# wfus/Fully-Homomorphic-Image-Processing

Hardware: AMD Instinct MI355X
Metric: encrypted 8x8 blocks/sec (homomorphic DCT+quant) (higher is better)
Workload: dtype f64

## Files before the change

### fully-homomorphic-image-processing_amd/csrc/dct_fused.hip

```cpp
#include "internal.h"

#include <cstdlib>

#include "fp64_core.h"

#pragma clang fp contract(off)

namespace {
using namespace fp64;

template <int L, int LE> struct Shape {
    static constexpr int N = 1 << L, E = 1 << LE, TP = N >> LE, NP = (L + LE - 1) / LE, LDS_WORDS = N + (N >> LE);
};
__host__ __device__ constexpr int g_lo(int L, int LE, int p) { return (L - LE * p - LE) < 0 ? 0 : (L - LE * p - LE); }
__host__ __device__ constexpr int g_stages(int L, int LE, int p) { return (L - LE * p) > LE ? LE : (L - LE * p); }
template <int LO, int LE> __device__ __forceinline__ int g_index(int tid, int r) {
    return ((tid >> LO) << (LO + LE)) | (r << LO) | (tid & ((1 << LO) - 1));
}
template <int LO, int LE> __device__ __forceinline__ int g_pad(int j) { return j + ((j >> (LO + LE)) << LO); }

template <int L, int LE, int P> struct PassTw {
    static constexpr int LO = g_lo(L, LE, P), S = g_stages(L, LE, P), NTW = (1 << LE) - 1;
    static constexpr int rb(int u) { return (L - 1 - (LE * P + u)) - LO; }
    static constexpr int count(int u) { return 1 << (LE - 1 - rb(u)); }
// ... 131 lines not shown
}
template <int L, int LE, int M, bool BIG, int P = Shape<L, LE>::NP - 1>
__device__ __forceinline__ void ntt_inv(double (&x)[M][1 << LE], double (&w)[(1 << LE) - 1], const double *__restrict__ itw, double p, double pinv,
                                        double *lds, int tid, int &phase) {
    if constexpr (P > 0) {
        double wn[(1 << LE) - 1];
        if (LE >= 4) load_tw<L, LE, P - 1>(wn, itw, tid);
        inv_pass<L, LE, P, M>(x, w, 0.0, p, pinv);
        if (LE < 4) load_tw<L, LE, P - 1>(wn, itw, tid);
        if constexpr (BIG) {
#pragma unroll
            for (int m = 0; m < M; m++)
#pragma unroll
                for (int r = 0; r < (1 << LE); r++) x[m][r] = red(x[m][r], p, pinv);
        }
        transpose<L, LE, g_lo(L, LE, P), g_lo(L, LE, P - 1), M>(x, lds, tid, phase);
        ntt_inv<L, LE, M, BIG, P - 1>(x, wn, itw, p, pinv, lds, tid, phase);
    } else {
        inv_pass<L, LE, P, M>(x, w, itw[0], p, pinv);
    }
}

constexpr double PACK_BIAS = 6755399441055744.0;
template <int E, int TP>
__device__ __forceinline__ void store_packed(char *__restrict__ ob, u32 vo, u32 so, const double (&x)[E]) {
    static_assert(E == 8, "packed layout is defined for 8 values per thread");
    u32 lo[8], hi[8];
#pragma unroll
    for (int r = 0; r < 8; r++) {
        const double t = x[r] + PACK_BIAS;
        lo[r] = (u32)__double2loint(t);
        hi[r] = (u32)__double2hiint(t);
    }
#pragma unroll
    for (int q = 0; q < 4; q++) *(u64 *)(ob + (size_t)(so + q * TP * 8) + vo) = (u64)lo[2 * q] | ((u64)lo[2 * q + 1] << 32);
    u32 h[2];
#pragma unroll
    for (int g = 0; g < 2; g++) {
        const u32 p01 = __builtin_amdgcn_perm(hi[4 * g + 1], hi[4 * g + 0], 0x0c0c0400u);
        const u32 p23 = __builtin_amdgcn_perm(hi[4 * g + 3], hi[4 * g + 2], 0x0c0c0400u);
        h[g] = __builtin_amdgcn_perm(p23, p01, 0x05040100u);
    }
    *(u64 *)(ob + (size_t)(so + 4 * TP * 8) + vo) = (u64)h[0] | ((u64)h[1] << 32);
}
typedef __attribute__((address_space(3))) void lc_lptr;
template <int NT>
__device__ __forceinline__ void stage_consts(gwin_t w, u32 voff, u32 soff, u32 cstride_bytes, double *stg) {
#pragma unroll
    for (int i0 = 0; i0 < NT; i0 += 2) {
        const int i = (i0 + 1 < NT) ? i0 : NT - 2;
        __builtin_amdgcn_raw_ptr_buffer_load_lds(w, (lc_lptr *)(stg + i * 64), 16, voff, soff + (u32)i * cstride_bytes, 0, 0);
    }
}

template <int L, int LE, bool BIG, int HALF, bool PACK, bool LDSC>
__device__ __forceinline__ void rows_body(const u64 *__restrict__ in, double *__restrict__ mid, const double *__restrict__ consts,
                                          const double *__restrict__ tw, const Work &wk, double p, double pinv, u32 k, double *lds) {
    using SH = Shape<L, LE>;
    constexpr int N = SH::N, TP = SH::TP, E = SH::E, NC = HalfC<HALF>::NC, FIRST = HalfC<HALF>::FIRST;
    const int tid = threadIdx.x;
    const size_t poly_words = (size_t)k * N, ct_words = 2 * poly_words;
    const size_t base = ((size_t)wk.blk * 64 + 8 * wk.line) * ct_words + (size_t)wk.poly * poly_words + (size_t)wk.prime * N;
    const gwin_t win_in = gwin(in + base), win_mid = gwin(mid + base);
    const u32 vo = (u32)tid * 8u, ctb = (u32)(ct_words * 8);
    double w0[E - 1];
    load_tw<L, LE, 0>(w0, tw, tid);
    double x[4][E];
    u64 ra[2][E], rb[2][E];
    auto issue = [&](int m) {
#pragma unroll
        for (int r = 0; r < E; r++) {
            ra[m & 1][r] = gld_u64(win_in, vo, (u32)m * ctb + r * TP * 8);
            rb[m & 1][r] = gld_u64(win_in, vo, (u32)(7 - m) * ctb + r * TP * 8);
        }
    };
// ... 45 lines not shown
    }
#pragma unroll
    for (int r = 0; r < E; r++) {
        double c[9];
        if constexpr (LDSC) {
            if (r + 1 < E) stage_consts<NC>(win_c, svoff, (r + 1) * TP * 8, csb, stg + ((r + 1) & 1) * NC * 64);
            if (r + 1 < E) asm volatile("s_waitcnt vmcnt(%0)" ::"n"(NDMA) : "memory");
            else asm volatile("s_waitcnt vmcnt(0)" ::: "memory");
            const double *sr = stg + (r & 1) * NC * 64 + lane;
#pragma unroll
            for (int i = 0; i < NC; i++) c[i] = sr[i * 64];
        } else {
        if (LE < 4) fetch(r);
#pragma unroll
        for (int i = 0; i < NC; i++) c[i] = cn[i];
        if (LE >= 4 && r + 1 < E) fetch(r + 1);
        }
        line_half<HALF>(x[0][r], x[1][r], x[2][r], x[3][r], c, p, pinv);
        if (BIG) {
#pragma unroll
            for (int m = 0; m < 4; m++) x[m][r] = red(x[m][r], p, pinv);
        } else if (PACK && HALF == 0) {
            x[0][r] = red(x[0][r], p, pinv);
            x[2][r] = red(x[2][r], p, pinv);
        }
        if constexpr (LDSC) asm volatile("" ::"v"(x[0][r]), "v"(x[1][r]), "v"(x[2][r]), "v"(x[3][r]) : "memory");
    }
#pragma unroll
    for (int m = 0; m < 4; m++) {
        const u32 so = (u32)(2 * m + HALF) * ctb;
        if constexpr (PACK) {
            store_packed<E, TP>((char *)(mid + base), vo, so, x[m]);
        } else {
#pragma unroll
            for (int r = 0; r < E; r++) gst_f64(win_mid, vo, so + r * TP * 8, x[m][r]);
        }
    }
}

__host__ __device__ constexpr int occ_waves(int tp, int lds_words) {
    return ((2 * lds_words * 16 <= 160 * 1024) ? 2 : 1) * tp / 256 < 1 ? 1 : ((2 * lds_words * 16 <= 160 * 1024) ? 2 : 1) * tp / 256;
}
template <int L, int LE> struct Occ { static constexpr int W = occ_waves(Shape<L, LE>::TP, Shape<L, LE>::LDS_WORDS); };

template <int L, int LE, bool BIG, bool PACK, bool LDSC>
__global__ __launch_bounds__((Shape<L, LE>::TP), (Occ<L, LE>::W)) void k_dct_rows(const u64 *__restrict__ in, double *__restrict__ mid,
                                                                  const double *__restrict__ consts, const double *__restrict__ tw_all,
                                                                  const Modulus *__restrict__ mods, u32 k) {
    __shared__ double lds[2 * Shape<L, LE>::LDS_WORDS];
    const Work wk = decode(blockIdx.x, k);
    const double p = (double)mods[wk.prime].q, pinv = 1.0 / p;
    const double *tw = tw_all + (size_t)wk.prime * Shape<L, LE>::N;
    if (wk.half) rows_body<L, LE, BIG, 1, PACK, LDSC>(in, mid, consts, tw, wk, p, pinv, k, lds);
    else rows_body<L, LE, BIG, 0, PACK, LDSC>(in, mid, consts, tw, wk, p, pinv, k, lds);
}

template <int L, int LE, bool BIG, int HALF, bool PACK>
__device__ __forceinline__ void cols_body(const double *__restrict__ mid, u64 *__restrict__ out, const double *__restrict__ consts,
                                          const double *__restrict__ itw, const Work &wk, double p, double pinv, u32 k, double *lds) {
    using SH = Shape<L, LE>;
    constexpr int N = SH::N, TP = SH::TP, E = SH::E, NC = HalfC<HALF>::NC, FIRST = HalfC<HALF>::FIRST;
    constexpr int LASTP = SH::NP - 1;
    const int tid = threadIdx.x;
    const size_t poly_words = (size_t)k * N, ct_words = 2 * poly_words;
    const size_t base = ((size_t)wk.blk * 64 + wk.line) * ct_words + (size_t)wk.poly * poly_words + (size_t)wk.prime * N;
    const size_t cstride = (size_t)k * N;
    const gwin_t win_mid = gwin(mid + base), win_out = gwin(out + base);
    const gwin_t win_c = gwin(consts + (size_t)FIRST * cstride + (size_t)wk.prime * N);
    const gwin_t win_s = gwin(consts + (size_t)(12 + 8 * HALF + wk.line) * cstride + (size_t)wk.prime * N);
    const u32 vo = (u32)tid * 8u, rsb = (u32)(ct_words * 64), csb = (u32)(cstride * 8);
    const double pbias = p + 4503599627370496.0;
    double cn[9], sn[4];
    auto fetch = [&](int r) {
#pragma unroll
        for (int i = 0; i < NC; i++) cn[i] = gld_f64(win_c, vo, (u32)i * csb + r * TP * 8);
#pragma unroll
        for (int m = 0; m < 4; m++) sn[m] = gld_f64(win_s, vo, (u32)(16 * m) * csb + r * TP * 8);
    };
    double wl[E - 1];
    if constexpr (!PACK) {
        fetch(0);
        load_tw<L, LE, LASTP>(wl, itw, tid);
    }
    double x[4][E];
    if constexpr (PACK) {
        u64 wa[4][5], wb[4][5];
#pragma unroll
        for (int m = 0; m < 4; m++) {
#pragma unroll
            for (int q = 0; q < 5; q++) {
                wa[m][q] = gld_u64(win_mid, vo, (u32)m * rsb + q * TP * 8);
                wb[m][q] = gld_u64(win_mid, vo, (u32)(7 - m) * rsb + q * TP * 8);
            }
        }
#pragma unroll
        for (int m = 0; m < 4; m++) {
#pragma unroll
            for (int r = 0; r < E; r++) {
                const u32 la = (r & 1) ? (u32)(wa[m][r >> 1] >> 32) : (u32)wa[m][r >> 1];
                const u32 lb = (r & 1) ? (u32)(wb[m][r >> 1] >> 32) : (u32)wb[m][r >> 1];
                const u32 hwa = (r & 4) ? (u32)(wa[m][4] >> 32) : (u32)wa[m][4], hwb = (r & 4) ? (u32)(wb[m][4] >> 32) : (u32)wb[m][4];
                const double ta = __hiloint2double((int)(0x43380000u + (u32)(int)(signed char)(hwa >> (8 * (r & 3)))), (int)la);
                const double tb = __hiloint2double((int)(0x43380000u + (u32)(int)(signed char)(hwb >> (8 * (r & 3)))), (int)lb);
                x[m][r] = HALF ? ta - tb : ta + (tb - 2.0 * PACK_BIAS);
            }
        }
    } else {
#pragma unroll
        for (int m = 0; m < 4; m++) {
#pragma unroll
            for (int r = 0; r < E; r++) {
                const double A = gld_f64(win_mid, vo, (u32)m * rsb + r * TP * 8), B = gld_f64(win_mid, vo, (u32)(7 - m) * rsb + r * TP * 8);
                x[m][r] = HALF ? A - B : A + B;
            }
        }
    }
    if constexpr (PACK) load_tw<L, LE, LASTP>(wl, itw, tid);
#pragma unroll
    for (int r = 0; r < E; r++) {
        double c[9], sc[4];
        if (PACK) fetch(r);
#pragma unroll
        for (int i = 0; i < NC; i++) c[i] = cn[i];
#pragma unroll
        for (int m = 0; m < 4; m++) sc[m] = sn[m];
        if (!PACK && r + 1 < E) fetch(r + 1);
        line_half<HALF>(x[0][r], x[1][r], x[2][r], x[3][r], c, p, pinv);
        double y[4] = {x[0][r], x[1][r], x[2][r], x[3][r]};
        mmv<4>(y, sc, p, pinv);
#pragma unroll
        for (int m = 0; m < 4; m++) x[m][r] = y[m];
    }
    int phase = 0;
    ntt_inv<L, LE, 4, BIG>(x, wl, itw, p, pinv, lds, tid, phase);
#pragma unroll
    for (int m = 0; m < 4; m++) {
#pragma unroll
        for (int r = 0; r < E; r++) gst_u64(win_out, vo, (u32)(2 * m + HALF) * rsb + r * TP * 8, f64_to_residue(x[m][r], pbias));
    }
}

template <int L, int LE, bool BIG, bool PACK>
__global__ __launch_bounds__((Shape<L, LE>::TP), (Occ<L, LE>::W)) void k_dct_cols(const double *__restrict__ mid, u64 *__restrict__ out,
                                                                  const double *__restrict__ consts, const double *__restrict__ itw_all,
                                                                  const Modulus *__restrict__ mods, u32 k) {
    __shared__ double lds[2 * Shape<L, LE>::LDS_WORDS];
    const Work wk = decode(blockIdx.x, k);
    const double p = (double)mods[wk.prime].q, pinv = 1.0 / p;
    const double *itw = itw_all + (size_t)wk.prime * Shape<L, LE>::N;
    if (wk.half) cols_body<L, LE, BIG, 1, PACK>(mid, out, consts, itw, wk, p, pinv, k, lds);
    else cols_body<L, LE, BIG, 0, PACK>(mid, out, consts, itw, wk, p, pinv, k, lds);
}

template <int L, int LE>
__global__ __launch_bounds__((Shape<L, LE>::TP), (Occ<L, LE>::W)) void k_dct_one_launch(const u64 *__restrict__ in, double *__restrict__ mid, u64 *__restrict__ out,
                                                                        const double *__restrict__ consts, const double *__restrict__ tw_all,
                                                                        const double *__restrict__ itw_all, const Modulus *__restrict__ mods, u32 k,
                                                                        u32 n_blocks, u32 dist, u32 *__restrict__ arrived, u32 *__restrict__ err) {
    __shared__ double lds[2 * Shape<L, LE>::LDS_WORDS];
    const u32 xcd = blockIdx.x & 7, seq = blockIdx.x >> 3, chunk = seq >> 5, r = seq & 31;
    const bool is_row = r < 16;
    const long j = is_row ? (long)chunk : (long)chunk - (long)(dist & 0xffffu);
    const u32 n_units = n_blocks * 2 * k;
    if (j < 0) return;
    const u64 g = (u64)j * 8 + xcd;
    if (g >= n_units) return;
    Work wk;
    wk.prime = (u32)(g / (n_blocks * 2));
    const u32 rem = (u32)(g - (u64)wk.prime * n_blocks * 2);
    wk.blk = rem >> 1;
    wk.poly = rem & 1;
    wk.line = (r & 15) >> 1;
    wk.half = r & 1;
    const double p = (double)mods[wk.prime].q, pinv = 1.0 / p;
    if (is_row) {
        const double *tw = tw_all + (size_t)wk.prime * Shape<L, LE>::N;
        if (wk.half) rows_body<L, LE, false, 1, true, true>(in, mid, consts, tw, wk, p, pinv, k, lds);
        else rows_body<L, LE, false, 0, true, true>(in, mid, consts, tw, wk, p, pinv, k, lds);
        if (dist & 0x10000u) return;
        __syncthreads();
        if (threadIdx.x == 0) {
            __threadfence();
            atomicAdd(arrived + g, 1u);
        }
    } else {
        if (!(dist & 0x10000u) && threadIdx.x == 0) {
            u32 spins = 0;
            while (__hip_atomic_load(arrived + g, __ATOMIC_RELAXED, __HIP_MEMORY_SCOPE_AGENT) < 16u) {
                __builtin_amdgcn_s_sleep(8);
                if (++spins > (1u << 24)) { atomicExch(err, 1u); break; }
            }
            __threadfence();
        }
        __syncthreads();
        const double *itw = itw_all + (size_t)wk.prime * Shape<L, LE>::N;
        if (wk.half) cols_body<L, LE, false, 1, true>(mid, out, consts, itw, wk, p, pinv, k, lds);
        else cols_body<L, LE, false, 0, true>(mid, out, consts, itw, wk, p, pinv, k, lds);
    }
}

__global__ void k_consts_to_f64(const ulonglong2 *__restrict__ in, double *__restrict__ out, const Modulus *__restrict__ mods, u32 k, u32 n, u32 le, u32 total) {
    const u32 i = blockIdx.x * blockDim.x + threadIdx.x;
    if (i >= total) return;
    const u32 pos = i % n, rowbase = i - pos;
    const u32 tp = n >> le, r = pos / tp, t = pos % tp;
    const u32 j = (t << le) + r;
    const u32 src = (j & 15) * (n >> 4) + (j >> 4);
    const u64 q = mods[(i / n) % k].q;
    const u64 w = in[rowbase + src].x;
    out[i] = w > q / 2 ? -(double)(q - w) : (double)w;
}

template <int L, int LE>
__global__ __launch_bounds__((Shape<L, LE>::TP), (Occ<L, LE>::W)) void k_rgb2ycc_f64(u64 *__restrict__ R, u64 *__restrict__ G, u64 *__restrict__ Bc,
                                                                     const double *__restrict__ consts, const double *__restrict__ tw_all,
                                                                     const double *__restrict__ itw_all, const Modulus *__restrict__ mods,
                                                                     const u64 *__restrict__ yoff, u32 yoff_len, u32 k, u32 group, u64 gstride) {
    using SH = Shape<L, LE>;
    constexpr int N = SH::N, TP = SH::TP, E = SH::E, LASTP = SH::NP - 1;
    __shared__ double lds[2 * SH::LDS_WORDS];
    const int tid = threadIdx.x;
    const u32 per_prime = gridDim.x / k;
    const u32 prime = blockIdx.x / per_prime;
    const u32 pp = blockIdx.x - prime * per_prime;
    const u32 poly = pp & 1, pix = pp >> 1;
    const u64 q = mods[prime].q;
    const double p = (double)q, pinv = 1.0 / p;
    const double *tw = tw_all + (size_t)prime * N, *itw = itw_all + (size_t)prime * N;
    const size_t pix_off = group ? (size_t)(pix / group) * gstride + (size_t)(pix % group) * 2 * k * N : (size_t)pix * 2 * k * N;
    const size_t off = pix_off + ((size_t)poly * k + prime) * N + tid;
    double w0[E - 1];
    load_tw<L, LE, 0>(w0, tw, tid);
    double x[3][E];
    {
        const u64 *src[3] = {R + off, G + off, Bc + off};
#pragma unroll
        for (int m = 0; m < 3; m++)
#pragma unroll
            for (int r = 0; r < E; r++) x[m][r] = u52_to_f64(src[m][r * TP]);
    }
    int phase = 0;
    ntt_fwd<L, LE, 3>(x, w0, tw, p, pinv, lds, tid, phase, [] {});
    double wl[E - 1];
// ... 88 lines not shown
            mmv<M>(y, wm, p, pinv);
#pragma unroll
            for (int m = 0; m < M; m++) x[m][r] = y[m];
        }
    }
    ntt_inv<L, LE, M, false>(x, wl, itw, p, pinv, lds, tid, phase);
#pragma unroll
    for (int m = 0; m < M; m++) {
        u64 *dst = out + ((size_t)(g * M + m) * k + prime) * N + tid;
#pragma unroll
        for (int r = 0; r < E; r++) {
            double v = x[m][r];
            v = v < 0.0 ? v + p : v;
            dst[r * TP] = f64_to_u52(v);
        }
    }
}

}


static u32 dct_shape_le(const fhe_ctx *c) {
    if (c->opt.dct_le != 3) return 4;
    if (c->logn == 12 && c->max_prime_bits <= 40) return 3;
    if (c->logn == 13 || c->logn == 11) return 3;
    return 4;
}

bool fhe_dct_f64_supported(const fhe_ctx *c) {
    return c && c->qb.d_tw_f64 && c->max_prime_bits <= 47 && (c->logn >= 10 && c->logn <= 13);
}

int fhe_dct_f64_make_consts(const fhe_ctx *c, fhe_dct_plan *plan, hipStream_t st) {
    const u32 total = DCT_NCONST * c->k * c->n;
    HIP_TRY(hipMalloc(&plan->d_consts_f64, sizeof(double) * total));
    const u32 le = dct_shape_le(c);
    k_consts_to_f64<<<(total + 255) / 256, 256, 0, st>>>(plan->d_consts, plan->d_consts_f64, c->qb.d_mod, c->k, c->n, le, total);
    KERNEL_CHECK();
    return FHE_OK;
}



template <int L, int LE>
static void launch_pair(const fhe_ctx *c, const fhe_dct_plan *plan, const u64 *in, u64 *out, double *mid, unsigned grid, bool big, hipStream_t st, int which) {
    constexpr int TP = Shape<L, LE>::TP;
    if constexpr (LE == 4) {
        if (big) {
            if (which & 1) k_dct_rows<L, LE, true, false, false><<<grid, TP, 0, st>>>(in, mid, plan->d_consts_f64, c->qb.d_tw_f64, c->qb.d_mod, c->k);
            if (which & 2) k_dct_cols<L, LE, true, false><<<grid, TP, 0, st>>>(mid, out, plan->d_consts_f64, c->qb.d_itw_f64, c->qb.d_mod, c->k);
            return;
        }
    }
    if constexpr (LE == 3) {
        if (big) {
            if (which & 1) k_dct_rows<L, LE, true, false, false><<<grid, TP, 0, st>>>(in, mid, plan->d_consts_f64, c->qb.d_tw_f64, c->qb.d_mod, c->k);
            if (which & 2) k_dct_cols<L, LE, true, false><<<grid, TP, 0, st>>>(mid, out, plan->d_consts_f64, c->qb.d_itw_f64, c->qb.d_mod, c->k);
            return;
        }
        if (c->max_prime_bits <= 37 && c->opt.dct_pack) {
            if (which & 1) {
                if (c->opt.dct_ldsc) k_dct_rows<L, LE, false, true, true><<<grid, TP, 0, st>>>(in, mid, plan->d_consts_f64, c->qb.d_tw_f64, c->qb.d_mod, c->k);
                else k_dct_rows<L, LE, false, true, false><<<grid, TP, 0, st>>>(in, mid, plan->d_consts_f64, c->qb.d_tw_f64, c->qb.d_mod, c->k);
            }
            if (which & 2) k_dct_cols<L, LE, false, true><<<grid, TP, 0, st>>>(mid, out, plan->d_consts_f64, c->qb.d_itw_f64, c->qb.d_mod, c->k);
            return;
        }
    }
    {
        if (which & 1) k_dct_rows<L, LE, false, false, false><<<grid, TP, 0, st>>>(in, mid, plan->d_consts_f64, c->qb.d_tw_f64, c->qb.d_mod, c->k);
        if (which & 2) k_dct_cols<L, LE, false, false><<<grid, TP, 0, st>>>(mid, out, plan->d_consts_f64, c->qb.d_itw_f64, c->qb.d_mod, c->k);
    }
}

int fhe_dct_f64_launch(const fhe_ctx *c, const fhe_dct_plan *plan, const u64 *in, u64 *out, u64 n_blocks, double *mid, hipStream_t st, int which) {
    const u64 items = n_blocks * 8 * 2 * c->k;
    const u64 grid = items * 2;
    if (grid > 0x7fffffffULL) return fail(FHE_ERR_PARAM, "too many blocks for one launch");
    if ((u64)c->k * c->n >= (1ULL << 21)) return fail(FHE_ERR_PARAM, "fused FP64 path: a block of ciphertexts exceeds the 2 GiB addressing window");
    const bool big = c->max_prime_bits > 40;
    if (c->opt.dct_one_launch && which == 3 && c->logn == 12 && dct_shape_le(c) == 3 && c->max_prime_bits <= 37 && c->opt.dct_pack && c->d_arrived) {
        const u64 n_units = n_blocks * 2 * c->k;
        if (n_units > c->arrived_cap) return fail(FHE_ERR_PARAM, "one-launch experiment: wave too large for the arrival counters");
        HIP_TRY(hipMemsetAsync(c->d_arrived, 0, (n_units + 1) * sizeof(u32), st));
        const u32 dist = c->opt.dct_one_launch;
        const u64 chunks = (n_units + 7) / 8 + (dist & 0xffffu);
        k_dct_one_launch<12, 3><<<(unsigned)(chunks * 32 * 8), Shape<12, 3>::TP, 0, st>>>(in, mid, out, plan->d_consts_f64, c->qb.d_tw_f64, c->qb.d_itw_f64, c->qb.d_mod,
                                                                                       c->k, (u32)n_blocks, dist, c->d_arrived + 1, c->d_arrived);
        KERNEL_CHECK();
        u32 timed_out = 0;
        HIP_TRY(hipMemcpyAsync(&timed_out, c->d_arrived, sizeof(u32), hipMemcpyDeviceToHost, st));
        HIP_TRY(hipStreamSynchronize(st));
        if (timed_out) return fail(FHE_ERR_HIP, "one-launch experiment: a column workgroup timed out waiting for its row transforms; the output is incomplete");
        return FHE_OK;
    }
    switch (c->logn) {
        case 10: launch_pair<10, 4>(c, plan, in, out, mid, (unsigned)grid, big, st, which); break;
        case 11: launch_pair<11, 3>(c, plan, in, out, mid, (unsigned)grid, big, st, which); break;
        case 12: if (dct_shape_le(c) == 3) launch_pair<12, 3>(c, plan, in, out, mid, (unsigned)grid, false, st, which); else launch_pair<12, 4>(c, plan, in, out, mid, (unsigned)grid, big, st, which); break;
        case 13: if (dct_shape_le(c) == 3) launch_pair<13, 3>(c, plan, in, out, mid, (unsigned)grid, big, st, which); else launch_pair<13, 4>(c, plan, in, out, mid, (unsigned)grid, big, st, which); break;
        default: return fail(FHE_ERR_PARAM, "fused FP64 path supports n in {1024, 2048, 4096, 8192}");
    }
    KERNEL_CHECK();
    return FHE_OK;
}

bool fhe_rgb_f64_supported(const fhe_ctx *c) {
    return fhe_dct_f64_supported(c) && c->logn == 12 && c->max_prime_bits <= 40;
}

int fhe_rgb_f64_make_consts(const fhe_ctx *c, const ulonglong2 *d_c, double **out, hipStream_t st) {
    const u32 total = 9 * c->k * c->n;
    HIP_TRY(hipMalloc(out, sizeof(double) * total));
    k_consts_to_f64<<<(total + 255) / 256, 256, 0, st>>>(d_c, *out, c->qb.d_mod, c->k, c->n, 3, total);
    KERNEL_CHECK();
    return FHE_OK;
}

int fhe_rgb_f64_launch(const fhe_ctx *c, u64 *r, u64 *g, u64 *b, u64 count, const double *consts, const u64 *yoff, u32 yoff_len, hipStream_t st, u32 group, u64 gstride) {
    const u64 grid = count * 2 * c->k;
// ... 195 lines not shown
```

### fully-homomorphic-image-processing_amd/csrc/fhe_hip.hip

```cpp
#include "internal.h"

#include <cmath>
#include <cstdarg>
#include <cstdio>
#include <cstdlib>
#include <cstring>
#include <algorithm>
#include <condition_variable>
#include <mutex>
#include <string>
#include <vector>

#include "host_math.h"

static thread_local std::string g_err;
int fhe_fail(int code, const char *fmt, ...) {
    char buf[512];
    va_list ap;
    va_start(ap, fmt);
    vsnprintf(buf, sizeof buf, fmt, ap);
    va_end(ap);
    g_err = buf;
    return code;
}
// ... 1284 lines not shown
    u64 *p = data + ((size_t)blk * 64 + (COLS ? line : 8 * line)) * ct_stride + ((size_t)poly * k + prime) * n + slot;
    const ulonglong2 *cp = consts + (size_t)prime * n + slot;
    const size_t cstride = (size_t)k * n;
    auto C = [&](int cid) { return cp[(size_t)cid * cstride]; };
    u64 v[8];
#pragma unroll
    for (int i = 0; i < 8; i++) v[i] = p[(size_t)i * step];
    if constexpr (!COLS) {
        dct_line_pm<1>(v, m, C);
#pragma unroll
        for (int i = 0; i < 8; i++) p[(size_t)i * step] = v[i];
    } else {
        dct_line_pm<24>(v, m, C);
#pragma unroll
        for (int i = 0; i < 8; i++) p[(size_t)i * step] = canon_pm(mulvv_pm(fold_pm(v[i], m), C(12 + 8 * i + line).x, m), m);
    }
}

extern "C" int fhe_dct_plan_create(const fhe_ctx *c, const double *quant64, int int_coeffs, int frac_coeffs, fhe_stream s, fhe_dct_plan **out) {
    if (!c || !out) return fail(FHE_ERR_PARAM, "null argument");
    *out = nullptr;
    fhe_dct_plan *p = new fhe_dct_plan();
    p->k = c->k;
    p->n = c->n;
    p->has_quant = quant64 != nullptr;
    const size_t pw = (size_t)c->k * c->n;
    int rc = fhe_dev_alloc(sizeof(ulonglong2) * pw * DCT_NCONST, (void **)&p->d_consts);
    if (rc) { delete p; return rc; }
    std::vector<uint64_t> plain(c->n);
    ulonglong2 *d_eighth = nullptr, *d_tmp = nullptr;
    auto cleanup = [&](int code) {
        if (d_eighth) (void)hipFree(d_eighth);
        if (d_tmp) (void)hipFree(d_tmp);
        if (code) { (void)hipFree(p->d_consts); if (p->d_consts_f64) (void)hipFree(p->d_consts_f64); if (p->d_consts_le3) (void)hipFree(p->d_consts_le3); delete p; }
        return code;
    };
    auto prep = [&](double v, ulonglong2 *dst) -> int {
        int len = fhe_frac_encode(c->n, c->t, v, int_coeffs, frac_coeffs, plain.data());
        if (len < 0) return len;
        return fhe_plain_prepare(c, plain.data(), (uint32_t)len, (uint64_t *)dst, s);
    };
    for (int i = 0; i < 12; ++i)
        if ((rc = prep(kDctConst[i], p->d_consts + pw * i))) return cleanup(rc);
    if (!quant64) {
        for (int i = 0; i < 64; ++i)
            if ((rc = prep(0.125, p->d_consts + pw * (12 + i)))) return cleanup(rc);
    } else {
        if ((rc = fhe_dev_alloc(sizeof(ulonglong2) * pw, (void **)&d_eighth))) return cleanup(rc);
        if ((rc = fhe_dev_alloc(sizeof(ulonglong2) * pw, (void **)&d_tmp))) return cleanup(rc);
        if ((rc = prep(0.125, d_eighth))) return cleanup(rc);
        for (int i = 0; i < 64; ++i) {
            if (!(quant64[i] != 0.0)) return cleanup(fail(FHE_ERR_PARAM, "quant[%d] is zero", i));
            if ((rc = prep(1 / quant64[i], d_tmp))) return cleanup(rc);
            if ((rc = fhe_plain_ntt_mul(c, (const uint64_t *)d_eighth, (const uint64_t *)d_tmp, (uint64_t *)(p->d_consts + pw * (12 + i)), s)))
                return cleanup(rc);
        }
    }
    if (fhe_dct_f64_supported(c) && (rc = fhe_dct_f64_make_consts(c, p, (hipStream_t)s))) return cleanup(rc);
    if (!fhe_dct_f64_supported(c) && fhe_dct_u64_supported(c) && (rc = fhe_dct_u64_make_consts(c, p, (hipStream_t)s))) return cleanup(rc);
    if (hipStreamSynchronize((hipStream_t)s) != hipSuccess) return cleanup(fail(FHE_ERR_HIP, "stream sync failed"));
    *out = p;
    return cleanup(FHE_OK);
}
extern "C" int fhe_dct_plan_destroy(fhe_dct_plan *p) {
    if (!p) return FHE_OK;
    if (p->d_consts) (void)hipFree(p->d_consts);
    if (p->d_consts_f64) (void)hipFree(p->d_consts_f64);
    if (p->d_consts_le3) (void)hipFree(p->d_consts_le3);
    delete p;
    return FHE_OK;
}
static u64 dct_wave_blocks(const fhe_ctx *c) { return c->opt.dct_wave_blocks; }
extern "C" size_t fhe_dct8x8_scratch_bytes(const fhe_ctx *c, uint64_t n_blocks) {
    if (!c || !(fhe_dct_f64_supported(c) || fhe_dct_u64_supported(c))) return 0;
    const u64 wave = dct_wave_blocks(c) < n_blocks ? dct_wave_blocks(c) : n_blocks;
    return (size_t)wave * 64 * 2 * c->k * c->n * sizeof(double);
}

extern "C" int fhe_dct_path(const fhe_ctx *c) {
    if (!c) return fail(FHE_ERR_PARAM, "null argument");
    if (fhe_dct_f64_supported(c) && !c->opt.force_u64) return 1;
    if (fhe_dct_u64_supported(c) && !c->opt.force_u64) return 2;
    return 0;
}

extern "C" int fhe_dct8x8_quant(const fhe_ctx *c, const fhe_dct_plan *plan, const uint64_t *in, uint64_t *out, uint64_t n_blocks,
                                void *scratch, size_t scratch_bytes, fhe_stream s) {
    if (!c || !plan || !in || !out) return fail(FHE_ERR_PARAM, "null argument");
    if (plan->k != c->k || plan->n != c->n) return fail(FHE_ERR_PARAM, "plan was built for another context");
    if (n_blocks == 0) return FHE_OK;
    hipStream_t st = (hipStream_t)s;
    if (plan->d_consts_f64 && fhe_dct_f64_supported(c) && !c->opt.force_u64) {
        const size_t per_block = (size_t)64 * 2 * c->k * c->n;
        const u64 fit = scratch ? scratch_bytes / (per_block * sizeof(double)) : 0;
        if (fit == 0) return fail(FHE_ERR_PARAM, "scratch too small: need fhe_dct8x8_scratch_bytes()");
        u64 wave = fit < dct_wave_blocks(c) ? fit : dct_wave_blocks(c);
        const bool pipelined = c->opt.dct_pipeline && fit >= 2 && n_blocks > wave / 2 && wave >= 2;
        if (!pipelined) {
            for (u64 b0 = 0; b0 < n_blocks; b0 += wave) {
                const u64 nb = (n_blocks - b0) < wave ? (n_blocks - b0) : wave;
                int rc = fhe_dct_f64_launch(c, plan, (const u64 *)in + b0 * per_block, (u64 *)out + b0 * per_block, nb, (double *)scratch, st);
                if (rc) return rc;
            }
            return FHE_OK;
        }
        const fhe_ctx *mc = c;
        wave = wave / 2 < 1 ? 1 : wave / 2;
        double *midbuf[2] = {(double *)scratch, (double *)scratch + wave * per_block};
        u64 w = 0;
        for (u64 b0 = 0; b0 < n_blocks; b0 += wave, ++w) {
            const u64 nb = (n_blocks - b0) < wave ? (n_blocks - b0) : wave;
            const int s = (int)(w & 1);
            if (w >= 2) HIP_TRY(hipStreamWaitEvent(st, mc->ev_cols[s], 0));
            int rc = fhe_dct_f64_launch(c, plan, (const u64 *)in + b0 * per_block, (u64 *)out + b0 * per_block, nb, midbuf[s], st, 1);
            if (rc) return rc;
            HIP_TRY(hipEventRecord(mc->ev_rows[s], st));
            HIP_TRY(hipStreamWaitEvent(mc->aux_stream, mc->ev_rows[s], 0));
            rc = fhe_dct_f64_launch(c, plan, (const u64 *)in + b0 * per_block, (u64 *)out + b0 * per_block, nb, midbuf[s], mc->aux_stream, 2);
            if (rc) return rc;
            HIP_TRY(hipEventRecord(mc->ev_cols[s], mc->aux_stream));
        }
        for (int s = 0; s < 2 && (u64)s < w; ++s) HIP_TRY(hipStreamWaitEvent(st, mc->ev_cols[s], 0));
        return FHE_OK;
    }
    if (plan->d_consts_le3 && fhe_dct_u64_supported(c) && !c->opt.force_u64) {
        const size_t per_block = (size_t)64 * 2 * c->k * c->n;
        const u64 fit = scratch ? scratch_bytes / (per_block * sizeof(u64)) : 0;
        if (fit == 0) return fail(FHE_ERR_PARAM, "scratch too small: need fhe_dct8x8_scratch_bytes()");
// ... 276 lines not shown
```

### fully-homomorphic-image-processing_amd/csrc/fp64_core.h

```cpp
#pragma once
#include "internal.h"

#pragma clang fp contract(off)

namespace fp64 {

__device__ __forceinline__ double mm(double y, double w, double p, double pinv) {
    const double h = y * w;
    const double l = __builtin_fma(y, w, -h);
    const double q = __builtin_rint(h * pinv);
    return __builtin_fma(-q, p, h) + l;
}
__device__ __forceinline__ double red(double x, double p, double pinv) {
    return __builtin_fma(-__builtin_rint(x * pinv), p, x);
}
template <int K>
__device__ __forceinline__ void mmv(double (&y)[K], const double (&w)[K], double p, double pinv) {
    double h[K], l[K], q[K];
#pragma unroll
    for (int i = 0; i < K; i++) h[i] = y[i] * w[i];
#pragma unroll
    for (int i = 0; i < K; i++) q[i] = h[i] * pinv;
#pragma unroll
    for (int i = 0; i < K; i++) l[i] = __builtin_fma(y[i], w[i], -h[i]);
#pragma unroll
    for (int i = 0; i < K; i++) q[i] = __builtin_rint(q[i]);
#pragma unroll
    for (int i = 0; i < K; i++) h[i] = __builtin_fma(-q[i], p, h[i]);
#pragma unroll
    for (int i = 0; i < K; i++) y[i] = h[i] + l[i];
}

__device__ __forceinline__ double u52_to_f64(u64 v) { return __longlong_as_double((long long)(v | 0x4330000000000000ULL)) - 4503599627370496.0; }
__device__ __forceinline__ u64 f64_to_u52(double v) { return (u64)__double_as_longlong(v + 4503599627370496.0) & 0x000FFFFFFFFFFFFFULL; }
__device__ __forceinline__ double u52_biased(u64 v) { return __longlong_as_double((long long)(v | 0x4330000000000000ULL)); }
__device__ __forceinline__ u64 f64_to_residue(double v, double pbias) {
    return (u64)__double_as_longlong(v + (v < 0.0 ? pbias : 4503599627370496.0)) & 0x000FFFFFFFFFFFFFULL;
}

typedef u32 u32x2 __attribute__((ext_vector_type(2)));
typedef __amdgpu_buffer_rsrc_t gwin_t;
__device__ __forceinline__ gwin_t gwin(const void *base) {
    return __builtin_amdgcn_make_buffer_rsrc(const_cast<void *>(base), 0, -1, 0x00020000 );
}
__device__ __forceinline__ u64 gld_u64(gwin_t w, u32 voff, u32 soff) { return __builtin_bit_cast(u64, __builtin_amdgcn_raw_buffer_load_b64(w, voff, soff, 0)); }
__device__ __forceinline__ double gld_f64(gwin_t w, u32 voff, u32 soff) { return __builtin_bit_cast(double, __builtin_amdgcn_raw_buffer_load_b64(w, voff, soff, 0)); }
__device__ __forceinline__ void gst_u64(gwin_t w, u32 voff, u32 soff, u64 v) { __builtin_amdgcn_raw_buffer_store_b64(__builtin_bit_cast(u32x2, v), w, voff, soff, 0); }
__device__ __forceinline__ void gst_f64(gwin_t w, u32 voff, u32 soff, double v) { __builtin_amdgcn_raw_buffer_store_b64(__builtin_bit_cast(u32x2, v), w, voff, soff, 0); }

template <int HALF>
__device__ __forceinline__ void line_half(double &x0, double &x1, double &x2, double &x3, const double (&c)[9], double p, double pinv) {
    if constexpr (HALF == 0) {
        const double tmp10 = x0 + x3, tmp13 = x0 - x3, tmp11 = x1 + x2, tmp12 = x1 - x2;
        double y[3] = {tmp12 + tmp13, tmp13, tmp12};
        const double w[3] = {c[0], c[1], c[2]};
        mmv<3>(y, w, p, pinv);
        x0 = tmp10 + tmp11;
        x2 = tmp10 - tmp11;
        x1 = y[0] + y[1];
        x3 = y[0] + y[2];
    } else {
        const double tmp7 = x0, tmp6 = x1, tmp5 = x2, tmp4 = x3;
        const double z1 = tmp4 + tmp7, z2 = tmp5 + tmp6, z3 = tmp4 + tmp6, z4 = tmp5 + tmp7;
        double ya[5] = {z3 + z4, tmp4, tmp5, tmp6, tmp7}, yb[4] = {z1, z2, z3, z4};
        const double wa[5] = {c[0], c[1], c[2], c[3], c[4]}, wb[4] = {c[5], c[6], c[7], c[8]};
        mmv<5>(ya, wa, p, pinv);
        mmv<4>(yb, wb, p, pinv);
        const double y[9] = {ya[0], ya[1], ya[2], ya[3], ya[4], yb[0], yb[1], yb[2], yb[3]};
        const double z3b = y[7] + y[0], z4b = y[8] + y[0];
        x0 = y[4] + y[5] + z4b;
        x1 = y[3] + y[6] + z3b;
        x2 = y[2] + y[6] + z4b;
        x3 = y[1] + y[5] + z3b;
    }
}
template <int HALF> struct HalfC { static constexpr int NC = HALF ? 9 : 3, FIRST = HALF ? 3 : 0; };

struct Work { u32 blk, line, poly, prime, half; };
__device__ __forceinline__ Work decode(u32 idx, u32 k) {
    const u32 w = ((idx >> 4) << 3) | (idx & 7);
    const u32 per_prime = (gridDim.x >> 1) / k;
// ... 14 lines not shown
```

### fully-homomorphic-image-processing_amd/csrc/internal.h

```cpp
#pragma once
#include "../../include/fhe_hip.h"

#include <hip/hip_runtime.h>

#include <mutex>
#include <string>
#include <vector>

#include "modarith.h"
#include "ntt_core.h"

int fhe_fail(int code, const char *fmt, ...) __attribute__((format(printf, 2, 3)));
#define fail fhe_fail
#define HIP_TRY(expr)                                                                             \
    do {                                                                                          \
        hipError_t e_ = (expr);                                                                   \
        if (e_ != hipSuccess) return fail(FHE_ERR_HIP, "%s: %s", #expr, hipGetErrorString(e_));   \
    } while (0)
#define KERNEL_CHECK()                                                                            \
    do {                                                                                          \
        hipError_t e_ = hipGetLastError();                                                        \
        if (e_ != hipSuccess) return fail(FHE_ERR_HIP, "kernel launch: %s", hipGetErrorString(e_)); \
    } while (0)

// ... 41 lines not shown

struct fhe_ctx {
    u32 n = 0, logn = 0, k = 0;
    FheOptions opt;
    u64 t = 0;
    int device = 0;
    int max_prime_bits = 0;
    BaseTables qb;
    u64 upper_half_threshold = 0;
    u64 plain_upper_half_increment[FHE_MAX_K] = {0};
    u64 delta_mod[FHE_MAX_K] = {0};
    u64 upper_half_increment[FHE_MAX_K] = {0};
    struct BehzTables *behz = nullptr;
    mutable std::once_flag behz_once;
    int behz_rc = 0;
    std::string behz_err;
    u32 *d_arrived = nullptr;
    u64 arrived_cap = 0;
    hipStream_t aux_stream = nullptr;
    hipEvent_t ev_rows[2] = {nullptr, nullptr}, ev_cols[2] = {nullptr, nullptr};
    struct RgbConsts {
        int int_coeffs = -1, frac_coeffs = -1;
        ulonglong2 *d_c = nullptr;
        double *d_c_f64 = nullptr;
        u64 *d_off = nullptr;
        u32 off_len = 0;
    };
    mutable std::vector<RgbConsts *> rgb;
    mutable std::vector<RgbConsts *> ycc;
    mutable std::mutex rgb_mutex;
};

#define DCT_NCONST 76
extern const double kDctConst[12];
struct fhe_dct_plan {
    ulonglong2 *d_consts = nullptr;
    double *d_consts_f64 = nullptr;
    ulonglong2 *d_consts_le3 = nullptr;
    u32 k = 0, n = 0;
    bool has_quant = false;
};

inline float fhe_resize_ref_coord(u32 i, u32 dst_len, u32 src_len) { return (float)((float)i / (float)(dst_len - 1) * (float)src_len - 0.5); }

#define DISPATCH_L(logn, ...)                                                    \
    switch (logn) {                                                              \
        case 10: { constexpr int L = 10; __VA_ARGS__; } break;                   \
        case 11: { constexpr int L = 11; __VA_ARGS__; } break;                   \
        case 12: { constexpr int L = 12; __VA_ARGS__; } break;                   \
        case 13: { constexpr int L = 13; __VA_ARGS__; } break;                   \
        case 14: { constexpr int L = 14; __VA_ARGS__; } break;                   \
        default: return fail(FHE_ERR_PARAM, "unsupported log2(n)=%u", logn);     \
    }

struct CMap {
    const u32 *idx;
    u64 div, cnt, off;
    __device__ __forceinline__ u64 operator()(u64 c) const { return idx ? idx[c] : (cnt ? ((off + c / div) % cnt) : c); }
};

#define FHE_PLAIN_SUM_MAX_TERMS 16
struct PlainSumTerms {
    u32 count;
    u32 size[FHE_PLAIN_SUM_MAX_TERMS];
    u64 *src[FHE_PLAIN_SUM_MAX_TERMS];
    const ulonglong2 *plain[FHE_PLAIN_SUM_MAX_TERMS];
};
bool fhe_multiply_plain_sum_supported(const fhe_ctx *c);
int fhe_multiply_plain_sum(const fhe_ctx *c, const PlainSumTerms &T, const u64 *addend, CMap amap, u32 addend_size, u64 *out, u32 out_size, u64 count,
                           hipStream_t st);
// ... 33 lines not shown
```

Baseline: 84630.

## Interleave mid and constant tables in pairs to use 128-bit buffer loads

Changes the intermediate row-pass output layout so adjacent element pairs sit contiguously, and builds a new paired constant table so the column pass can fetch two doubles per 128-bit buffer load instead of two 64-bit loads. The packed path reads the low words with b128 loads, and twiddle loading is moved after the constant multiply. This aims to halve the number of memory instructions in the column kernel and widen accesses. In exchange it adds a second constant table (more memory and setup work) and a 16-byte alignment adjustment for the scratch buffer.

```diff
diff --git a/fully-homomorphic-image-processing_amd/csrc/dct_fused.hip b/fully-homomorphic-image-processing_amd/csrc/dct_fused.hip
--- a/fully-homomorphic-image-processing_amd/csrc/dct_fused.hip
+++ b/fully-homomorphic-image-processing_amd/csrc/dct_fused.hip
@@ -187,8 +187,6 @@
         lo[r] = (u32)__double2loint(t);
         hi[r] = (u32)__double2hiint(t);
     }
-#pragma unroll
-    for (int q = 0; q < 4; q++) *(u64 *)(ob + (size_t)(so + q * TP * 8) + vo) = (u64)lo[2 * q] | ((u64)lo[2 * q + 1] << 32);
     u32 h[2];
 #pragma unroll
     for (int g = 0; g < 2; g++) {
@@ -196,6 +194,8 @@
         const u32 p23 = __builtin_amdgcn_perm(hi[4 * g + 3], hi[4 * g + 2], 0x0c0c0400u);
         h[g] = __builtin_amdgcn_perm(p23, p01, 0x05040100u);
     }
+#pragma unroll
+    for (int q = 0; q < 4; q++) *(u64 *)(ob + (size_t)(so + (q >> 1) * TP * 16 + (q & 1) * 8) + 2 * vo) = (u64)lo[2 * q] | ((u64)lo[2 * q + 1] << 32);
     *(u64 *)(ob + (size_t)(so + 4 * TP * 8) + vo) = (u64)h[0] | ((u64)h[1] << 32);
 }
 typedef __attribute__((address_space(3))) void lc_lptr;
@@ -307,8 +307,13 @@
         if constexpr (PACK) {
             store_packed<E, TP>((char *)(mid + base), vo, so, x[m]);
         } else {
-#pragma unroll
-            for (int r = 0; r < E; r++) gst_f64(win_mid, vo, so + r * TP * 8, x[m][r]);
+            if constexpr (LE >= 4) {
+#pragma unroll
+                for (int r = 0; r < E; r++) gst_f64(win_mid, 2 * vo, so + (r >> 1) * TP * 16 + (r & 1) * 8, x[m][r]);
+            } else {
+#pragma unroll
+                for (int j = 0; j < E / 2; j++) gst_f64x2(win_mid, 2 * vo, so + j * TP * 16, x[m][2 * j], x[m][2 * j + 1]);
+            }
         }
     }
 }
@@ -332,7 +337,7 @@
 
 template <int L, int LE, bool BIG, int HALF, bool PACK>
 __device__ __forceinline__ void cols_body(const double *__restrict__ mid, u64 *__restrict__ out, const double *__restrict__ consts,
-                                          const double *__restrict__ itw, const Work &wk, double p, double pinv, u32 k, double *lds) {
+                                          const double *__restrict__ cpairs, const double *__restrict__ itw, const Work &wk, double p, double pinv, u32 k, double *lds) {
     using SH = Shape<L, LE>;
     constexpr int N = SH::N, TP = SH::TP, E = SH::E, NC = HalfC<HALF>::NC, FIRST = HalfC<HALF>::FIRST;
     constexpr int LASTP = SH::NP - 1;
@@ -341,16 +346,35 @@
     const size_t base = ((size_t)wk.blk * 64 + wk.line) * ct_words + (size_t)wk.poly * poly_words + (size_t)wk.prime * N;
     const size_t cstride = (size_t)k * N;
     const gwin_t win_mid = gwin(mid + base), win_out = gwin(out + base);
-    const gwin_t win_c = gwin(consts + (size_t)FIRST * cstride + (size_t)wk.prime * N);
-    const gwin_t win_s = gwin(consts + (size_t)(12 + 8 * HALF + wk.line) * cstride + (size_t)wk.prime * N);
+    const gwin_t win_c = PACK ? gwin(cpairs + 2 * ((size_t)(HALF ? 1 : 0) * cstride + (size_t)wk.prime * N))
+                              : gwin(consts + (size_t)FIRST * cstride + (size_t)wk.prime * N);
+    const gwin_t win_s = PACK ? gwin(cpairs + 2 * ((size_t)(DCT_NPAIR_LINE + 2 * (2 * wk.line + HALF)) * cstride + (size_t)wk.prime * N))
+                              : gwin(consts + (size_t)(12 + 8 * HALF + wk.line) * cstride + (size_t)wk.prime * N);
+    const gwin_t win_1 = gwin(consts + (size_t)(FIRST + NC - 1) * cstride + (size_t)wk.prime * N);
     const u32 vo = (u32)tid * 8u, rsb = (u32)(ct_words * 64), csb = (u32)(cstride * 8);
     const double pbias = p + 4503599627370496.0;
     double cn[9], sn[4];
     auto fetch = [&](int r) {
-#pragma unroll
-        for (int i = 0; i < NC; i++) cn[i] = gld_f64(win_c, vo, (u32)i * csb + r * TP * 8);
-#pragma unroll
-        for (int m = 0; m < 4; m++) sn[m] = gld_f64(win_s, vo, (u32)(16 * m) * csb + r * TP * 8);
+        if constexpr (PACK) {
+#pragma unroll
+            for (int i = 0; i < NC / 2; i++) {
+                const f64x2 v = gld_f64x2(win_c, 2 * vo, (u32)i * 2 * csb + r * TP * 16);
+                cn[2 * i] = v.a;
+                cn[2 * i + 1] = v.b;
+            }
+            cn[NC - 1] = gld_f64(win_1, vo, r * TP * 8);
+#pragma unroll
+            for (int g = 0; g < 2; g++) {
+                const f64x2 v = gld_f64x2(win_s, 2 * vo, (u32)g * 2 * csb + r * TP * 16);
+                sn[2 * g] = v.a;
+                sn[2 * g + 1] = v.b;
+            }
+        } else {
+#pragma unroll
+            for (int i = 0; i < NC; i++) cn[i] = gld_f64(win_c, vo, (u32)i * csb + r * TP * 8);
+#pragma unroll
+            for (int m = 0; m < 4; m++) sn[m] = gld_f64(win_s, vo, (u32)(16 * m) * csb + r * TP * 8);
+        }
     };
     double wl[E - 1];
     if constexpr (!PACK) {
@@ -359,24 +383,25 @@
     }
     double x[4][E];
     if constexpr (PACK) {
-        u64 wa[4][5], wb[4][5];
+        u32x4 qa[4][2], qb[4][2];
+        u64 ha[4], hb[4];
 #pragma unroll
         for (int m = 0; m < 4; m++) {
 #pragma unroll
-            for (int q = 0; q < 5; q++) {
-                wa[m][q] = gld_u64(win_mid, vo, (u32)m * rsb + q * TP * 8);
-                wb[m][q] = gld_u64(win_mid, vo, (u32)(7 - m) * rsb + q * TP * 8);
-            }
+            for (int g = 0; g < 2; g++) {
+                qa[m][g] = gld_b128(win_mid, 2 * vo, (u32)m * rsb + g * TP * 16);
+                qb[m][g] = gld_b128(win_mid, 2 * vo, (u32)(7 - m) * rsb + g * TP * 16);
+            }
+            ha[m] = gld_u64(win_mid, vo, (u32)m * rsb + 4 * TP * 8);
+            hb[m] = gld_u64(win_mid, vo, (u32)(7 - m) * rsb + 4 * TP * 8);
         }
 #pragma unroll
         for (int m = 0; m < 4; m++) {
 #pragma unroll
             for (int r = 0; r < E; r++) {
-                const u32 la = (r & 1) ? (u32)(wa[m][r >> 1] >> 32) : (u32)wa[m][r >> 1];
-                const u32 lb = (r & 1) ? (u32)(wb[m][r >> 1] >> 32) : (u32)wb[m][r >> 1];
-                const u32 hwa = (r & 4) ? (u32)(wa[m][4] >> 32) : (u32)wa[m][4], hwb = (r & 4) ? (u32)(wb[m][4] >> 32) : (u32)wb[m][4];
-                const double ta = __hiloint2double((int)(0x43380000u + (u32)(int)(signed char)(hwa >> (8 * (r & 3)))), (int)la);
-                const double tb = __hiloint2double((int)(0x43380000u + (u32)(int)(signed char)(hwb >> (8 * (r & 3)))), (int)lb);
+                const u32 hwa = (r & 4) ? (u32)(ha[m] >> 32) : (u32)ha[m], hwb = (r & 4) ? (u32)(hb[m] >> 32) : (u32)hb[m];
+                const double ta = __hiloint2double((int)(0x43380000u + (u32)(int)(signed char)(hwa >> (8 * (r & 3)))), (int)qa[m][r >> 2][r & 3]);
+                const double tb = __hiloint2double((int)(0x43380000u + (u32)(int)(signed char)(hwb >> (8 * (r & 3)))), (int)qb[m][r >> 2][r & 3]);
                 x[m][r] = HALF ? ta - tb : ta + (tb - 2.0 * PACK_BIAS);
             }
         }
@@ -384,13 +409,13 @@
 #pragma unroll
         for (int m = 0; m < 4; m++) {
 #pragma unroll
-            for (int r = 0; r < E; r++) {
-                const double A = gld_f64(win_mid, vo, (u32)m * rsb + r * TP * 8), B = gld_f64(win_mid, vo, (u32)(7 - m) * rsb + r * TP * 8);
-                x[m][r] = HALF ? A - B : A + B;
-            }
-        }
-    }
-    if constexpr (PACK) load_tw<L, LE, LASTP>(wl, itw, tid);
+            for (int j = 0; j < E / 2; j++) {
+                const f64x2 A = gld_f64x2(win_mid, 2 * vo, (u32)m * rsb + j * TP * 16), B = gld_f64x2(win_mid, 2 * vo, (u32)(7 - m) * rsb + j * TP * 16);
+                x[m][2 * j] = HALF ? A.a - B.a : A.a + B.a;
+                x[m][2 * j + 1] = HALF ? A.b - B.b : A.b + B.b;
+            }
+        }
+    }
 #pragma unroll
     for (int r = 0; r < E; r++) {
         double c[9], sc[4];
@@ -406,6 +431,7 @@
 #pragma unroll
         for (int m = 0; m < 4; m++) x[m][r] = y[m];
     }
+    if constexpr (PACK) load_tw<L, LE, LASTP>(wl, itw, tid);
     int phase = 0;
     ntt_inv<L, LE, 4, BIG>(x, wl, itw, p, pinv, lds, tid, phase);
 #pragma unroll
@@ -417,19 +443,19 @@
 
 template <int L, int LE, bool BIG, bool PACK>
 __global__ __launch_bounds__((Shape<L, LE>::TP), (Occ<L, LE>::W)) void k_dct_cols(const double *__restrict__ mid, u64 *__restrict__ out,
-                                                                  const double *__restrict__ consts, const double *__restrict__ itw_all,
+                                                                  const double *__restrict__ consts, const double *__restrict__ cpairs, const double *__restrict__ itw_all,
                                                                   const Modulus *__restrict__ mods, u32 k) {
     __shared__ double lds[2 * Shape<L, LE>::LDS_WORDS];
     const Work wk = decode(blockIdx.x, k);
     const double p = (double)mods[wk.prime].q, pinv = 1.0 / p;
     const double *itw = itw_all + (size_t)wk.prime * Shape<L, LE>::N;
-    if (wk.half) cols_body<L, LE, BIG, 1, PACK>(mid, out, consts, itw, wk, p, pinv, k, lds);
-    else cols_body<L, LE, BIG, 0, PACK>(mid, out, consts, itw, wk, p, pinv, k, lds);
+    if (wk.half) cols_body<L, LE, BIG, 1, PACK>(mid, out, consts, cpairs, itw, wk, p, pinv, k, lds);
+    else cols_body<L, LE, BIG, 0, PACK>(mid, out, consts, cpairs, itw, wk, p, pinv, k, lds);
 }
 
 template <int L, int LE>
 __global__ __launch_bounds__((Shape<L, LE>::TP), (Occ<L, LE>::W)) void k_dct_one_launch(const u64 *__restrict__ in, double *__restrict__ mid, u64 *__restrict__ out,
-                                                                        const double *__restrict__ consts, const double *__restrict__ tw_all,
+                                                                        const double *__restrict__ consts, const double *__restrict__ cpairs, const double *__restrict__ tw_all,
                                                                         const double *__restrict__ itw_all, const Modulus *__restrict__ mods, u32 k,
                                                                         u32 n_blocks, u32 dist, u32 *__restrict__ arrived, u32 *__restrict__ err) {
     __shared__ double lds[2 * Shape<L, LE>::LDS_WORDS];
@@ -469,8 +495,8 @@
         }
         __syncthreads();
         const double *itw = itw_all + (size_t)wk.prime * Shape<L, LE>::N;
-        if (wk.half) cols_body<L, LE, false, 1, true>(mid, out, consts, itw, wk, p, pinv, k, lds);
-        else cols_body<L, LE, false, 0, true>(mid, out, consts, itw, wk, p, pinv, k, lds);
+        if (wk.half) cols_body<L, LE, false, 1, true>(mid, out, consts, cpairs, itw, wk, p, pinv, k, lds);
+        else cols_body<L, LE, false, 0, true>(mid, out, consts, cpairs, itw, wk, p, pinv, k, lds);
     }
 }
 
@@ -484,6 +510,28 @@
     const u64 q = mods[(i / n) % k].q;
     const u64 w = in[rowbase + src].x;
     out[i] = w > q / 2 ? -(double)(q - w) : (double)w;
+}
+
+__global__ void k_consts_to_pairs(const ulonglong2 *__restrict__ in, double *__restrict__ out, const Modulus *__restrict__ mods, u32 k, u32 n, u32 le, u32 total) {
+    const u32 i = blockIdx.x * blockDim.x + threadIdx.x;
+    if (i >= total) return;
+    const u32 pos = i % n, prime = (i / n) % k, pt = i / (n * k);
+    const u32 tp = n >> le, r = pos / tp, t = pos % tp;
+    const u32 j = (t << le) + r;
+    const u32 src = (j & 15) * (n >> 4) + (j >> 4);
+    u32 ca, cb;
+    if (pt < DCT_NPAIR_LINE) {
+        ca = pt ? 2 * pt + 1 : 0;
+        cb = ca + 1;
+    } else {
+        const u32 u = pt - DCT_NPAIR_LINE, g = u & 1, half = (u >> 1) & 1, col = u >> 2;
+        ca = 12 + 8 * (4 * g + half) + col;
+        cb = ca + 16;
+    }
+    const u64 q = mods[prime].q;
+    const u64 wa = in[((size_t)ca * k + prime) * n + src].x, wb = in[((size_t)cb * k + prime) * n + src].x;
+    out[2 * (size_t)i] = wa > q / 2 ? -(double)(q - wa) : (double)wa;
+    out[2 * (size_t)i + 1] = wb > q / 2 ? -(double)(q - wb) : (double)wb;
 }
 
 template <int L, int LE>
@@ -638,11 +686,17 @@
 }
 
 int fhe_dct_f64_make_consts(const fhe_ctx *c, fhe_dct_plan *plan, hipStream_t st) {
-    const u32 total = DCT_NCONST * c->k * c->n;
+    const u32 total = DCT_NCONST * c->k * c->n, pairs = DCT_NPAIR * c->k * c->n;
+    const u32 le = dct_shape_le(c);
+    const bool packed = c->max_prime_bits <= 37 && le == 3 && c->opt.dct_pack;
     HIP_TRY(hipMalloc(&plan->d_consts_f64, sizeof(double) * total));
-    const u32 le = dct_shape_le(c);
+    if (packed) { HIP_TRY(hipMalloc(&plan->d_consts_pair, 2 * sizeof(double) * pairs)); }
     k_consts_to_f64<<<(total + 255) / 256, 256, 0, st>>>(plan->d_consts, plan->d_consts_f64, c->qb.d_mod, c->k, c->n, le, total);
     KERNEL_CHECK();
+    if (packed) {
+        k_consts_to_pairs<<<(pairs + 255) / 256, 256, 0, st>>>(plan->d_consts, plan->d_consts_pair, c->qb.d_mod, c->k, c->n, le, pairs);
+        KERNEL_CHECK();
+    }
     return FHE_OK;
 }
 
@@ -654,14 +708,14 @@
     if constexpr (LE == 4) {
         if (big) {
             if (which & 1) k_dct_rows<L, LE, true, false, false><<<grid, TP, 0, st>>>(in, mid, plan->d_consts_f64, c->qb.d_tw_f64, c->qb.d_mod, c->k);
-            if (which & 2) k_dct_cols<L, LE, true, false><<<grid, TP, 0, st>>>(mid, out, plan->d_consts_f64, c->qb.d_itw_f64, c->qb.d_mod, c->k);
+            if (which & 2) k_dct_cols<L, LE, true, false><<<grid, TP, 0, st>>>(mid, out, plan->d_consts_f64, plan->d_consts_pair, c->qb.d_itw_f64, c->qb.d_mod, c->k);
             return;
         }
     }
     if constexpr (LE == 3) {
         if (big) {
             if (which & 1) k_dct_rows<L, LE, true, false, false><<<grid, TP, 0, st>>>(in, mid, plan->d_consts_f64, c->qb.d_tw_f64, c->qb.d_mod, c->k);
-            if (which & 2) k_dct_cols<L, LE, true, false><<<grid, TP, 0, st>>>(mid, out, plan->d_consts_f64, c->qb.d_itw_f64, c->qb.d_mod, c->k);
+            if (which & 2) k_dct_cols<L, LE, true, false><<<grid, TP, 0, st>>>(mid, out, plan->d_consts_f64, plan->d_consts_pair, c->qb.d_itw_f64, c->qb.d_mod, c->k);
             return;
         }
         if (c->max_prime_bits <= 37 && c->opt.dct_pack) {
@@ -669,13 +723,13 @@
                 if (c->opt.dct_ldsc) k_dct_rows<L, LE, false, true, true><<<grid, TP, 0, st>>>(in, mid, plan->d_consts_f64, c->qb.d_tw_f64, c->qb.d_mod, c->k);
                 else k_dct_rows<L, LE, false, true, false><<<grid, TP, 0, st>>>(in, mid, plan->d_consts_f64, c->qb.d_tw_f64, c->qb.d_mod, c->k);
             }
-            if (which & 2) k_dct_cols<L, LE, false, true><<<grid, TP, 0, st>>>(mid, out, plan->d_consts_f64, c->qb.d_itw_f64, c->qb.d_mod, c->k);
+            if (which & 2) k_dct_cols<L, LE, false, true><<<grid, TP, 0, st>>>(mid, out, plan->d_consts_f64, plan->d_consts_pair, c->qb.d_itw_f64, c->qb.d_mod, c->k);
             return;
         }
     }
     {
         if (which & 1) k_dct_rows<L, LE, false, false, false><<<grid, TP, 0, st>>>(in, mid, plan->d_consts_f64, c->qb.d_tw_f64, c->qb.d_mod, c->k);
-        if (which & 2) k_dct_cols<L, LE, false, false><<<grid, TP, 0, st>>>(mid, out, plan->d_consts_f64, c->qb.d_itw_f64, c->qb.d_mod, c->k);
+        if (which & 2) k_dct_cols<L, LE, false, false><<<grid, TP, 0, st>>>(mid, out, plan->d_consts_f64, plan->d_consts_pair, c->qb.d_itw_f64, c->qb.d_mod, c->k);
     }
 }
 
@@ -685,13 +739,15 @@
     if (grid > 0x7fffffffULL) return fail(FHE_ERR_PARAM, "too many blocks for one launch");
     if ((u64)c->k * c->n >= (1ULL << 21)) return fail(FHE_ERR_PARAM, "fused FP64 path: a block of ciphertexts exceeds the 2 GiB addressing window");
     const bool big = c->max_prime_bits > 40;
+    if (!big && dct_shape_le(c) == 3 && c->max_prime_bits <= 37 && c->opt.dct_pack && !plan->d_consts_pair)
+        return fail(FHE_ERR_PARAM, "fused FP64 path: the plan has no paired constant tables (it was created for a context without the packed intermediate)");
     if (c->opt.dct_one_launch && which == 3 && c->logn == 12 && dct_shape_le(c) == 3 && c->max_prime_bits <= 37 && c->opt.dct_pack && c->d_arrived) {
         const u64 n_units = n_blocks * 2 * c->k;
         if (n_units > c->arrived_cap) return fail(FHE_ERR_PARAM, "one-launch experiment: wave too large for the arrival counters");
         HIP_TRY(hipMemsetAsync(c->d_arrived, 0, (n_units + 1) * sizeof(u32), st));
         const u32 dist = c->opt.dct_one_launch;
         const u64 chunks = (n_units + 7) / 8 + (dist & 0xffffu);
-        k_dct_one_launch<12, 3><<<(unsigned)(chunks * 32 * 8), Shape<12, 3>::TP, 0, st>>>(in, mid, out, plan->d_consts_f64, c->qb.d_tw_f64, c->qb.d_itw_f64, c->qb.d_mod,
+        k_dct_one_launch<12, 3><<<(unsigned)(chunks * 32 * 8), Shape<12, 3>::TP, 0, st>>>(in, mid, out, plan->d_consts_f64, plan->d_consts_pair, c->qb.d_tw_f64, c->qb.d_itw_f64, c->qb.d_mod,
                                                                                        c->k, (u32)n_blocks, dist, c->d_arrived + 1, c->d_arrived);
         KERNEL_CHECK();
         u32 timed_out = 0;
diff --git a/fully-homomorphic-image-processing_amd/csrc/fhe_hip.hip b/fully-homomorphic-image-processing_amd/csrc/fhe_hip.hip
--- a/fully-homomorphic-image-processing_amd/csrc/fhe_hip.hip
+++ b/fully-homomorphic-image-processing_amd/csrc/fhe_hip.hip
@@ -1340,7 +1340,7 @@
     auto cleanup = [&](int code) {
         if (d_eighth) (void)hipFree(d_eighth);
         if (d_tmp) (void)hipFree(d_tmp);
-        if (code) { (void)hipFree(p->d_consts); if (p->d_consts_f64) (void)hipFree(p->d_consts_f64); if (p->d_consts_le3) (void)hipFree(p->d_consts_le3); delete p; }
+        if (code) { (void)hipFree(p->d_consts); if (p->d_consts_f64) (void)hipFree(p->d_consts_f64); if (p->d_consts_pair) (void)hipFree(p->d_consts_pair); if (p->d_consts_le3) (void)hipFree(p->d_consts_le3); delete p; }
         return code;
     };
     auto prep = [&](double v, ulonglong2 *dst) -> int {
@@ -1374,6 +1374,7 @@
     if (!p) return FHE_OK;
     if (p->d_consts) (void)hipFree(p->d_consts);
     if (p->d_consts_f64) (void)hipFree(p->d_consts_f64);
+    if (p->d_consts_pair) (void)hipFree(p->d_consts_pair);
     if (p->d_consts_le3) (void)hipFree(p->d_consts_le3);
     delete p;
     return FHE_OK;
@@ -1382,7 +1383,7 @@
 extern "C" size_t fhe_dct8x8_scratch_bytes(const fhe_ctx *c, uint64_t n_blocks) {
     if (!c || !(fhe_dct_f64_supported(c) || fhe_dct_u64_supported(c))) return 0;
     const u64 wave = dct_wave_blocks(c) < n_blocks ? dct_wave_blocks(c) : n_blocks;
-    return (size_t)wave * 64 * 2 * c->k * c->n * sizeof(double);
+    return (size_t)wave * 64 * 2 * c->k * c->n * sizeof(double) + 16;
 }
 
 extern "C" int fhe_dct_path(const fhe_ctx *c) {
@@ -1400,8 +1401,10 @@
     hipStream_t st = (hipStream_t)s;
     if (plan->d_consts_f64 && fhe_dct_f64_supported(c) && !c->opt.force_u64) {
         const size_t per_block = (size_t)64 * 2 * c->k * c->n;
-        const u64 fit = scratch ? scratch_bytes / (per_block * sizeof(double)) : 0;
+        const size_t lost = scratch ? (size_t)(-(uintptr_t)scratch & 15) : 0;
+        const u64 fit = scratch && scratch_bytes > lost ? (scratch_bytes - lost) / (per_block * sizeof(double)) : 0;
         if (fit == 0) return fail(FHE_ERR_PARAM, "scratch too small: need fhe_dct8x8_scratch_bytes()");
+        scratch = (char *)scratch + lost;
         u64 wave = fit < dct_wave_blocks(c) ? fit : dct_wave_blocks(c);
         const bool pipelined = c->opt.dct_pipeline && fit >= 2 && n_blocks > wave / 2 && wave >= 2;
         if (!pipelined) {
diff --git a/fully-homomorphic-image-processing_amd/csrc/fp64_core.h b/fully-homomorphic-image-processing_amd/csrc/fp64_core.h
--- a/fully-homomorphic-image-processing_amd/csrc/fp64_core.h
+++ b/fully-homomorphic-image-processing_amd/csrc/fp64_core.h
@@ -47,6 +47,13 @@
 __device__ __forceinline__ double gld_f64(gwin_t w, u32 voff, u32 soff) { return __builtin_bit_cast(double, __builtin_amdgcn_raw_buffer_load_b64(w, voff, soff, 0)); }
 __device__ __forceinline__ void gst_u64(gwin_t w, u32 voff, u32 soff, u64 v) { __builtin_amdgcn_raw_buffer_store_b64(__builtin_bit_cast(u32x2, v), w, voff, soff, 0); }
 __device__ __forceinline__ void gst_f64(gwin_t w, u32 voff, u32 soff, double v) { __builtin_amdgcn_raw_buffer_store_b64(__builtin_bit_cast(u32x2, v), w, voff, soff, 0); }
+typedef u32 u32x4 __attribute__((ext_vector_type(4)));
+struct f64x2 { double a, b; };
+__device__ __forceinline__ u32x4 gld_b128(gwin_t w, u32 voff, u32 soff) { return __builtin_amdgcn_raw_buffer_load_b128(w, voff, soff, 0); }
+__device__ __forceinline__ f64x2 gld_f64x2(gwin_t w, u32 voff, u32 soff) { return __builtin_bit_cast(f64x2, __builtin_amdgcn_raw_buffer_load_b128(w, voff, soff, 0)); }
+__device__ __forceinline__ void gst_f64x2(gwin_t w, u32 voff, u32 soff, double a, double b) {
+    __builtin_amdgcn_raw_buffer_store_b128(__builtin_bit_cast(u32x4, f64x2{a, b}), w, voff, soff, 0);
+}
 
 template <int HALF>
 __device__ __forceinline__ void line_half(double &x0, double &x1, double &x2, double &x3, const double (&c)[9], double p, double pinv) {
diff --git a/fully-homomorphic-image-processing_amd/csrc/internal.h b/fully-homomorphic-image-processing_amd/csrc/internal.h
--- a/fully-homomorphic-image-processing_amd/csrc/internal.h
+++ b/fully-homomorphic-image-processing_amd/csrc/internal.h
@@ -97,10 +97,13 @@
 };
 
 #define DCT_NCONST 76
+#define DCT_NPAIR_LINE 5
+#define DCT_NPAIR (DCT_NPAIR_LINE + 32)
 extern const double kDctConst[12];
 struct fhe_dct_plan {
     ulonglong2 *d_consts = nullptr;
     double *d_consts_f64 = nullptr;
+    double *d_consts_pair = nullptr;
     ulonglong2 *d_consts_le3 = nullptr;
     u32 k = 0, n = 0;
     bool has_quant = false;
```

Result: faster. 89460 (median of 6 runs) (+5.7%).
